# Transconnectome/multimodal_neuroimage

Measured on NVIDIA B200. Metric: window_attn_fwd_bwd, higher is better.
Workload: dtype bf16

## Files before the change

### multimodal_neuroimage_b200/csrc/tc_common.cuh

```cuda
#pragma once

#include <cuda.h>
#include <cuda_bf16.h>
#include <cuda_runtime.h>
#include <stdint.h>
#include <stdio.h>

namespace mmn { namespace tc {

__device__ __forceinline__ uint32_t smem_u32(const void* p) { return (uint32_t)__cvta_generic_to_shared(p); }

__device__ __forceinline__ void mbar_init(uint64_t* bar, uint32_t count) {
  asm volatile("mbarrier.init.shared::cta.b64 [%0], %1;" ::"r"(smem_u32(bar)), "r"(count));
}
__device__ __forceinline__ void fence_barrier_init() { asm volatile("fence.mbarrier_init.release.cluster;" ::: "memory"); }
__device__ __forceinline__ void mbar_arrive(uint64_t* bar) {
  asm volatile("mbarrier.arrive.shared::cta.b64 _, [%0];" ::"r"(smem_u32(bar)) : "memory");
}
__device__ __forceinline__ void mbar_arrive_warp(uint64_t* bar) {
  __syncwarp();
  if ((threadIdx.x & 31) == 0) mbar_arrive(bar);
}
__device__ __forceinline__ void mbar_arrive_expect_tx(uint64_t* bar, uint32_t bytes) {
  asm volatile("mbarrier.arrive.expect_tx.shared::cta.b64 _, [%0], %1;" ::"r"(smem_u32(bar)), "r"(bytes) : "memory");
}
__device__ __forceinline__ bool mbar_try_wait(uint64_t* bar, uint32_t parity) {
  uint32_t ok;
  asm volatile(
      "{\n\t.reg .pred p;\n\t"
      "mbarrier.try_wait.parity.shared::cta.b64 p, [%1], %2, %3;\n\t"
      "selp.u32 %0, 1, 0, p;\n\t}"
      : "=r"(ok)
      : "r"(smem_u32(bar)), "r"(parity), "r"(0x989680u)
      : "memory");
  return ok != 0;
}
__device__ __forceinline__ bool mbar_test(uint64_t* bar, uint32_t parity) {
  uint32_t ok;
  asm volatile(
      "{\n\t.reg .pred p;\n\t"
      "mbarrier.test_wait.parity.shared::cta.b64 p, [%1], %2;\n\t"
      "selp.u32 %0, 1, 0, p;\n\t}"
      : "=r"(ok)
      : "r"(smem_u32(bar)), "r"(parity)
      : "memory");
  return ok != 0;
}
__device__ __forceinline__ void mbar_wait(uint64_t* bar, uint32_t parity) {
  uint32_t spins = 0;
  while (!mbar_try_wait(bar, parity)) {
    if (++spins > (1u << 20)) {
#ifdef MMN_DEBUG_WAIT
      printf("mbar_wait timeout: block %d thread %d barrier smem 0x%x parity %u\n", (int)blockIdx.x, (int)threadIdx.x, smem_u32(bar), parity);
#endif
      __trap();
    }
  }
}

__device__ __forceinline__ bool elect_one() {
  uint32_t pred;
  asm volatile("{\n\t.reg .pred p;\n\telect.sync _|p, 0xffffffff;\n\tselp.u32 %0, 1, 0, p;\n\t}" : "=r"(pred));
  return pred != 0;
}

__device__ __forceinline__ void fence_proxy_async_smem() { asm volatile("fence.proxy.async.shared::cta;" ::: "memory"); }
__device__ __forceinline__ void tcgen05_fence_before() { asm volatile("tcgen05.fence::before_thread_sync;" ::: "memory"); }
__device__ __forceinline__ void tcgen05_fence_after() { asm volatile("tcgen05.fence::after_thread_sync;" ::: "memory"); }
__device__ __forceinline__ void named_bar_sync(uint32_t id, uint32_t threads) {
  asm volatile("bar.sync %0, %1;" ::"r"(id), "r"(threads) : "memory");
}

__device__ __forceinline__ void tma_prefetch_desc(const CUtensorMap* m) {
  asm volatile("prefetch.tensormap [%0];" ::"l"(reinterpret_cast<uint64_t>(m)) : "memory");
}
__device__ __forceinline__ void tma_load_5d(const CUtensorMap* m, uint64_t* bar, void* smem_dst, int c0, int c1, int c2,
                                            int c3, int c4) {
  asm volatile(
      "cp.async.bulk.tensor.5d.shared::cluster.global.mbarrier::complete_tx::bytes [%0], [%1, {%3, %4, %5, %6, %7}], [%2];"
      ::"r"(smem_u32(smem_dst)), "l"(reinterpret_cast<uint64_t>(m)), "r"(smem_u32(bar)), "r"(c0), "r"(c1), "r"(c2),
      "r"(c3), "r"(c4)
      : "memory");
}
__device__ __forceinline__ void tma_store_5d(const CUtensorMap* m, const void* smem_src, int c0, int c1, int c2, int c3,
                                             int c4) {
  asm volatile("cp.async.bulk.tensor.5d.global.shared::cta.bulk_group [%0, {%2, %3, %4, %5, %6}], [%1];" ::"l"(
                   reinterpret_cast<uint64_t>(m)),
               "r"(smem_u32(smem_src)), "r"(c0), "r"(c1), "r"(c2), "r"(c3), "r"(c4)
               : "memory");
}
__device__ __forceinline__ void tma_load_3d(const CUtensorMap* m, uint64_t* bar, void* smem_dst, int c0, int c1, int c2) {
  asm volatile(
      "cp.async.bulk.tensor.3d.shared::cluster.global.mbarrier::complete_tx::bytes [%0], [%1, {%3, %4, %5}], [%2];"
      ::"r"(smem_u32(smem_dst)), "l"(reinterpret_cast<uint64_t>(m)), "r"(smem_u32(bar)), "r"(c0), "r"(c1), "r"(c2)
      : "memory");
}
__device__ __forceinline__ void tma_load_4d(const CUtensorMap* m, uint64_t* bar, void* smem_dst, int c0, int c1, int c2, int c3) {
  asm volatile(
      "cp.async.bulk.tensor.4d.shared::cluster.global.mbarrier::complete_tx::bytes [%0], [%1, {%3, %4, %5, %6}], [%2];"
      ::"r"(smem_u32(smem_dst)), "l"(reinterpret_cast<uint64_t>(m)), "r"(smem_u32(bar)), "r"(c0), "r"(c1), "r"(c2), "r"(c3)
      : "memory");
}
__device__ __forceinline__ void tma_prefetch_3d(const CUtensorMap* m, int c0, int c1, int c2) {
  asm volatile("cp.async.bulk.prefetch.tensor.3d.L2.global.tile [%0, {%1, %2, %3}];" ::"l"(reinterpret_cast<uint64_t>(m)), "r"(c0),
               "r"(c1), "r"(c2)
               : "memory");
}
__device__ __forceinline__ void tma_store_3d(const CUtensorMap* m, const void* smem_src, int c0, int c1, int c2) {
  asm volatile("cp.async.bulk.tensor.3d.global.shared::cta.bulk_group [%0, {%2, %3, %4}], [%1];" ::"l"(
                   reinterpret_cast<uint64_t>(m)),
               "r"(smem_u32(smem_src)), "r"(c0), "r"(c1), "r"(c2)
               : "memory");
}
__device__ __forceinline__ void bulk_load_1d(void* smem_dst, const void* gsrc, uint32_t bytes, uint64_t* bar) {
  asm volatile("cp.async.bulk.shared::cluster.global.mbarrier::complete_tx::bytes [%0], [%1], %2, [%3];" ::"r"(smem_u32(smem_dst)),
               "l"(reinterpret_cast<uint64_t>(gsrc)), "r"(bytes), "r"(smem_u32(bar))
               : "memory");
}
__device__ __forceinline__ void tma_store_commit() { asm volatile("cp.async.bulk.commit_group;" ::: "memory"); }
template <int N>
__device__ __forceinline__ void tma_store_wait_read() { asm volatile("cp.async.bulk.wait_group.read %0;" ::"n"(N) : "memory"); }
template <int N>
__device__ __forceinline__ void tma_store_wait_all() { asm volatile("cp.async.bulk.wait_group %0;" ::"n"(N) : "memory"); }

template <int COLS>
__device__ __forceinline__ void tmem_alloc(uint32_t* dst_smem) {
  asm volatile("tcgen05.alloc.cta_group::1.sync.aligned.shared::cta.b32 [%0], %1;" ::"r"(smem_u32(dst_smem)), "n"(COLS)
               : "memory");
  asm volatile("tcgen05.relinquish_alloc_permit.cta_group::1.sync.aligned;" ::: "memory");
}
template <int COLS>
__device__ __forceinline__ void tmem_dealloc(uint32_t taddr) {
  asm volatile("tcgen05.dealloc.cta_group::1.sync.aligned.b32 %0, %1;" ::"r"(taddr), "n"(COLS) : "memory");
}
__device__ __forceinline__ void tmem_ld_wait() { asm volatile("tcgen05.wait::ld.sync.aligned;" ::: "memory"); }

__device__ __forceinline__ void tmem_ld_32x32b_x32(uint32_t taddr, uint32_t (&r)[32]) {
  asm volatile(
      "tcgen05.ld.sync.aligned.32x32b.x32.b32 "
      "{%0, %1, %2, %3, %4, %5, %6, %7, %8, %9, %10, %11, %12, %13, %14, %15, "
      "%16, %17, %18, %19, %20, %21, %22, %23, %24, %25, %26, %27, %28, %29, %30, %31}, [%32];"
      : "=r"(r[0]), "=r"(r[1]), "=r"(r[2]), "=r"(r[3]), "=r"(r[4]), "=r"(r[5]), "=r"(r[6]), "=r"(r[7]), "=r"(r[8]),
        "=r"(r[9]), "=r"(r[10]), "=r"(r[11]), "=r"(r[12]), "=r"(r[13]), "=r"(r[14]), "=r"(r[15]), "=r"(r[16]),
        "=r"(r[17]), "=r"(r[18]), "=r"(r[19]), "=r"(r[20]), "=r"(r[21]), "=r"(r[22]), "=r"(r[23]), "=r"(r[24]),
        "=r"(r[25]), "=r"(r[26]), "=r"(r[27]), "=r"(r[28]), "=r"(r[29]), "=r"(r[30]), "=r"(r[31])
      : "r"(taddr)
      : "memory");
}

__device__ __forceinline__ void tmem_ld_32x32b_x16(uint32_t taddr, uint32_t (&r)[16]) {
  asm volatile(
      "tcgen05.ld.sync.aligned.32x32b.x16.b32 "
      "{%0, %1, %2, %3, %4, %5, %6, %7, %8, %9, %10, %11, %12, %13, %14, %15}, [%16];"
      : "=r"(r[0]), "=r"(r[1]), "=r"(r[2]), "=r"(r[3]), "=r"(r[4]), "=r"(r[5]), "=r"(r[6]), "=r"(r[7]), "=r"(r[8]),
        "=r"(r[9]), "=r"(r[10]), "=r"(r[11]), "=r"(r[12]), "=r"(r[13]), "=r"(r[14]), "=r"(r[15])
      : "r"(taddr)
      : "memory");
}

__device__ __forceinline__ void tmem_ld_32x32b(uint32_t taddr, uint32_t (&r)[16]) { tmem_ld_32x32b_x16(taddr, r); }
__device__ __forceinline__ void tmem_ld_32x32b(uint32_t taddr, uint32_t (&r)[32]) { tmem_ld_32x32b_x32(taddr, r); }

__device__ __forceinline__ void tmem_st_32x32b_x32(uint32_t taddr, const uint32_t (&r)[32]) {
  asm volatile(
      "tcgen05.st.sync.aligned.32x32b.x32.b32 [%0], "
      "{%1, %2, %3, %4, %5, %6, %7, %8, %9, %10, %11, %12, %13, %14, %15, %16, "
      "%17, %18, %19, %20, %21, %22, %23, %24, %25, %26, %27, %28, %29, %30, %31, %32};"
      ::"r"(taddr), "r"(r[0]), "r"(r[1]), "r"(r[2]), "r"(r[3]), "r"(r[4]), "r"(r[5]), "r"(r[6]), "r"(r[7]), "r"(r[8]), "r"(r[9]),
      "r"(r[10]), "r"(r[11]), "r"(r[12]), "r"(r[13]), "r"(r[14]), "r"(r[15]), "r"(r[16]), "r"(r[17]), "r"(r[18]), "r"(r[19]),
      "r"(r[20]), "r"(r[21]), "r"(r[22]), "r"(r[23]), "r"(r[24]), "r"(r[25]), "r"(r[26]), "r"(r[27]), "r"(r[28]), "r"(r[29]),
      "r"(r[30]), "r"(r[31])
      : "memory");
}
__device__ __forceinline__ void tmem_st_32x32b_x16(uint32_t taddr, const uint32_t (&r)[16]) {
  asm volatile(
      "tcgen05.st.sync.aligned.32x32b.x16.b32 [%0], "
      "{%1, %2, %3, %4, %5, %6, %7, %8, %9, %10, %11, %12, %13, %14, %15, %16};"
      ::"r"(taddr), "r"(r[0]), "r"(r[1]), "r"(r[2]), "r"(r[3]), "r"(r[4]), "r"(r[5]), "r"(r[6]), "r"(r[7]), "r"(r[8]), "r"(r[9]),
      "r"(r[10]), "r"(r[11]), "r"(r[12]), "r"(r[13]), "r"(r[14]), "r"(r[15])
      : "memory");
}
__device__ __forceinline__ void tmem_st_wait() { asm volatile("tcgen05.wait::st.sync.aligned;" ::: "memory"); }

template <int R> __device__ __forceinline__ void setmaxnreg_inc() { asm volatile("setmaxnreg.inc.sync.aligned.u32 %0;" ::"n"(R)); }
template <int R> __device__ __forceinline__ void setmaxnreg_dec() { asm volatile("setmaxnreg.dec.sync.aligned.u32 %0;" ::"n"(R)); }

enum : uint64_t { kSwzNone = 0, kSwz128 = 2, kSwz64 = 4, kSwz32 = 6 };
__device__ __forceinline__ uint64_t umma_smem_desc(uint32_t saddr, uint32_t lbo_bytes, uint32_t sbo_bytes, uint64_t layout) {
  return (uint64_t)((saddr & 0x3FFFF) >> 4) | ((uint64_t)(lbo_bytes >> 4) << 16) | ((uint64_t)(sbo_bytes >> 4) << 32) |
         (1ull << 46) | (layout << 61);
}
__host__ __device__ constexpr uint32_t umma_idesc_bf16(int M, int N, int a_mn_major, int b_mn_major) {
  return (1u << 4) | (1u << 7) | (1u << 10) | ((uint32_t)a_mn_major << 15) | ((uint32_t)b_mn_major << 16) |
         ((uint32_t)(N >> 3) << 17) | ((uint32_t)(M >> 4) << 24);
}
__device__ __forceinline__ void umma_bf16_ss(uint32_t tmem_d, uint64_t adesc, uint64_t bdesc, uint32_t idesc, uint32_t accumulate) {
  asm volatile(
      "{\n\t.reg .pred p;\n\t"
      "setp.ne.b32 p, %4, 0;\n\t"
      "tcgen05.mma.cta_group::1.kind::f16 [%0], %1, %2, %3, p;\n\t}"
      ::"r"(tmem_d), "l"(adesc), "l"(bdesc), "r"(idesc), "r"(accumulate)
      : "memory");
}
__device__ __forceinline__ void umma_bf16_ts(uint32_t tmem_d, uint32_t tmem_a, uint64_t bdesc, uint32_t idesc, uint32_t accumulate) {
  asm volatile(
      "{\n\t.reg .pred p;\n\t"
      "setp.ne.b32 p, %4, 0;\n\t"
      "tcgen05.mma.cta_group::1.kind::f16 [%0], [%1], %2, %3, p;\n\t}"
      ::"r"(tmem_d), "r"(tmem_a), "l"(bdesc), "r"(idesc), "r"(accumulate)
      : "memory");
}
__device__ __forceinline__ void umma_commit(uint64_t* bar) {
  asm volatile("tcgen05.commit.cta_group::1.mbarrier::arrive::one.shared::cluster.b64 [%0];" ::"r"(smem_u32(bar)) : "memory");
}

__device__ __forceinline__ uint32_t pack_bf16x2(float lo, float hi) {
  __nv_bfloat162 v = __floats2bfloat162_rn(lo, hi);
  return *reinterpret_cast<uint32_t*>(&v);
}
__device__ __forceinline__ uint64_t pk2(float lo, float hi) {
  uint64_t r;
  asm("mov.b64 %0, {%1, %2};" : "=l"(r) : "f"(lo), "f"(hi));
  return r;
}
__device__ __forceinline__ uint64_t pk2u(uint32_t lo, uint32_t hi) {
  uint64_t r;
  asm("mov.b64 %0, {%1, %2};" : "=l"(r) : "r"(lo), "r"(hi));
  return r;
}
__device__ __forceinline__ void upk2(uint64_t v, float& lo, float& hi) { asm("mov.b64 {%0, %1}, %2;" : "=f"(lo), "=f"(hi) : "l"(v)); }
__device__ __forceinline__ uint64_t fma2(uint64_t a, uint64_t b, uint64_t c) {
  uint64_t r;
  asm("fma.rn.f32x2 %0, %1, %2, %3;" : "=l"(r) : "l"(a), "l"(b), "l"(c));
  return r;
}
__device__ __forceinline__ uint64_t mul2(uint64_t a, uint64_t b) {
  uint64_t r;
  asm("mul.rn.f32x2 %0, %1, %2;" : "=l"(r) : "l"(a), "l"(b));
  return r;
}
__device__ __forceinline__ uint64_t add2(uint64_t a, uint64_t b) {
  uint64_t r;
  asm("add.rn.f32x2 %0, %1, %2;" : "=l"(r) : "l"(a), "l"(b));
  return r;
}
__device__ __forceinline__ uint32_t pack_bf16x2(uint64_t v) {
  float lo, hi;
  upk2(v, lo, hi);
  return pack_bf16x2(lo, hi);
}
__device__ __forceinline__ float fast_exp2(float x) {
  float y;
  asm("ex2.approx.ftz.f32 %0, %1;" : "=f"(y) : "f"(x));
  return y;
}

}}
```

### multimodal_neuroimage_b200/csrc/winattn_tc_bwd.cuh

```cuda
#pragma once

#include "winattn_tc_fwd.cuh"

namespace mmn { namespace tc {

constexpr int kStagesB = 3;
constexpr int kStageBytesB = 2 * kQRegion + 2 * kTile;
constexpr int kOffK = kQRegion, kOffV = kQRegion + kTile, kOffDO = kQRegion + 2 * kTile;
#ifndef MMN_BWD_KEYS_PER_THREAD
#define MMN_BWD_KEYS_PER_THREAD 16
#endif
constexpr int kKeysPerThread = MMN_BWD_KEYS_PER_THREAD;
constexpr int kRowSplit = kN / kKeysPerThread;
constexpr int kSoftmaxThreadsB = 128 * kRowSplit, kEpiThreads = 128;
constexpr int kEpiWarp0 = kSoftmaxThreadsB / 32, kProducerWarpB = kEpiWarp0 + 4, kMmaWarpB = kEpiWarp0 + 5, kStoreWarpB = kEpiWarp0 + 6;
constexpr int kColsumWarpB = kEpiWarp0 + 7;
constexpr int kBwdThreads = kSoftmaxThreadsB + 256;
constexpr int kRegLaunch = kRowSplit == 4 ? 80 : 128;
constexpr int kRegSoftmax = kRowSplit == 4 ? 80 : 168, kRegEpi = kRowSplit == 4 ? 104 : 112, kRegAux = kRowSplit == 4 ? 56 : 64;
#ifndef MMN_BWD_CHUNK
#define MMN_BWD_CHUNK 1
#endif
constexpr int kChunkB = MMN_BWD_CHUNK;
constexpr int kPDBytes = 7 * 8192;
constexpr int kBwdTmemCols = 512;

struct BwdParams {
  CUtensorMap q[8], k[8], v[8], dout[8], dq[8], dk[8], dv[8];
  WinShape S;
  Sched sc;
  int nH, per_head;
  int mask_windows;
  float scale;
  const float* bias;
  const float* head_scale;
  const float* mask;
  const float* lse;
  long long slab;
  float* dbias;
  float* dhead_scale;
  float* dcolsum;
  int* work;
  float* part;
  TraceCfg trace;
};


constexpr int kDetColsum = kN * kN, kDetHscale = kN * kN + 3 * kD, kDetSlotFloats = kN * kN + 3 * kD + 4;

template <bool COS, int MASK, bool DET>
__global__ void __launch_bounds__(kBwdThreads, 1)
winattn_bwd_tc_kernel(const __grid_constant__ BwdParams P) {
  extern __shared__ uint8_t smem_raw[];
  uint8_t* smem = smem_raw + ((1024u - (smem_u32(smem_raw) & 1023u)) & 1023u);
  uint8_t* sStage = smem;
  uint8_t* sPD = sStage + kStagesB * kStageBytesB;
  uint8_t* sDS = sPD + 2 * 8192;
  uint8_t* sOut = sPD + kPDBytes;
  float* sTbl = reinterpret_cast<float*>(sOut + 3 * kTile);
  float* sRec = sTbl + kN * kTblLd;
  float* sDelta = sRec + kStagesB * 2 * 3 * kN;
  float* sRed = sDelta + 512;
  uint8_t* sPos = reinterpret_cast<uint8_t*>(sRed + 16);
  uint8_t* sRid = sPos + 512;
  int4* sItem = reinterpret_cast<int4*>(sRid + 512);
  int4* sGeo = sItem + 8;
  int* sEnd = reinterpret_cast<int*>(sGeo + 16);
  uint64_t* bars = reinterpret_cast<uint64_t*>(sEnd + 4);
  uint64_t* full = bars;
  uint64_t* empty = bars + kStagesB;
  uint64_t* sdp_full = bars + 2 * kStagesB;
  uint64_t* sdp_empty = sdp_full + 2;
  uint64_t* pds_full = sdp_full + 4;
  uint64_t* out_full = sdp_full + 5;
  uint64_t* out_empty = sdp_full + 7;
  uint64_t* so_ready = sdp_full + 9;
  uint64_t* so_free = sdp_full + 12;
  uint32_t* tmem_slot = reinterpret_cast<uint32_t*>(sdp_full + 15);

  const WinShape& S = P.S;
  const Sched& sc = P.sc;
  const int tid = threadIdx.x, warp = tid >> 5, lane = tid & 31;
  const int h = blockIdx.x % P.nH;
  float* const det_slot = DET ? P.part + (size_t)(h * P.per_head + blockIdx.x / P.nH) * kDetSlotFloats : nullptr;

  for (int i = tid; i < (kStagesB * kStageBytesB + kPDBytes) / 16; i += kBwdThreads)
    reinterpret_cast<uint4*>(smem)[i] = make_uint4(0, 0, 0, 0);
  for (int i = tid; i < 512; i += kBwdThreads) {
    sPos[i] = (uint8_t)piece_position(S, i >> 6, i & 63);
    sRid[i] = (uint8_t)class_region_id(S, i >> 6, i & 63);
  }
  for (int i = tid; i < kStagesB * 2 * 3 * kN; i += kBwdThreads) sRec[i] = 0.f;
  if (tid == 0) {
    sEnd[0] = 0x7fffffff;
    for (int s = 0; s < kStagesB; ++s) { mbar_init(&full[s], 1); mbar_init(&empty[s], kEpiThreads / 32); }
    for (int b = 0; b < 2; ++b) {
      mbar_init(&sdp_full[b], 1); mbar_init(&sdp_empty[b], kSoftmaxThreadsB / 32);
      mbar_init(&out_full[b], 1); mbar_init(&out_empty[b], kEpiThreads / 32);
    }
    mbar_init(pds_full, kSoftmaxThreadsB / 32);
    for (int t = 0; t < 3; ++t) { mbar_init(&so_ready[t], kEpiThreads / 32); mbar_init(&so_free[t], P.dcolsum ? 2 : 1); }
    fence_barrier_init();
  }
  if (warp == kProducerWarpB && lane == 0)
    for (int i = 0; i < 8; ++i) { tma_prefetch_desc(&P.q[i]); tma_prefetch_desc(&P.k[i]); tma_prefetch_desc(&P.v[i]); tma_prefetch_desc(&P.dout[i]); }
  if (warp == kStoreWarpB && lane == 0)
    for (int i = 0; i < 8; ++i) { tma_prefetch_desc(&P.dq[i]); tma_prefetch_desc(&P.dk[i]); tma_prefetch_desc(&P.dv[i]); }
  if (warp == kMmaWarpB) tmem_alloc<kBwdTmemCols>(tmem_slot);
  fence_proxy_async_smem();
  tcgen05_fence_before();
  __syncthreads();
  tcgen05_fence_after();
  const uint32_t tmem = *tmem_slot;
  trace_cta_time(P.trace, 0);

  if (warp >= kProducerWarpB) {
    setmaxnreg_dec<kRegAux>();
    if (warp == kProducerWarpB) {
      const CUtensorMap* const maps[4] = {P.q, P.dout, P.k, P.v};
      const int dst_base[4] = {0, kOffDO, kOffK, kOffV};
      const int slot_stride[4] = {2 * kWinBytes, 2 * kWinBytes, kWinBytes, kWinBytes};
      BoxPlan<4> plan;
      int n = 0;
#define MMN_BWD_LOAD_ITEM(cur)                                                                                           \
  do {                                                                                                                 \
    const int stage = n % kStagesB, phase = (n / kStagesB) & 1;                                                       \
    if ((cur).cls != plan.cls) plan.build(S, (cur).cls, lane, maps, dst_base, slot_stride);                           \
    const int nvalid = (cur).slot_valid(1) ? 2 : 1;                                                                   \
    int w0, w1;                                                                                                       \
    const WinStart ws0 = cursor_start(S, cur, 0, w0), ws1 = cursor_start(S, cur, 1, w1);                              \
    trace_ev(P.trace, 2, n, 0);                                                                                       \
    mbar_wait(&empty[stage], phase ^ 1);                                                                              \
    trace_ev(P.trace, 2, n, 1);                                                                                       \
    if (lane == 0) {                                                                                                  \
      sItem[n & 7] = make_int4((cur).cls, w0, w1, nvalid);                                                          \
      sGeo[(n & 7) * 2] = make_int4(ws0.b, ws0.s0, ws0.s1, ws0.s2);                                                   \
      sGeo[(n & 7) * 2 + 1] = make_int4(ws1.b, ws1.s0, ws1.s1, ws1.s2);                                               \
      mbar_arrive_expect_tx(&full[stage], nvalid * (4 * kWinBytes + 3 * kN * 4));                                     \
    }                                                                                                                 \
    __syncwarp();                                                                                                     \
    plan.issue<true>(S, ws0, ws1, nvalid, h * kD, sStage + stage * kStageBytesB, &full[stage], lane);                 \
    if (lane < nvalid)                                                                                                \
      bulk_load_1d(sRec + (stage * 2 + lane) * (3 * kN), P.lse + P.slab + ((long long)(lane ? w1 : w0) * P.nH + h) * (3 * kN),\
                   3 * kN * 4, &full[stage]);                                                                         \
    trace_ev(P.trace, 2, n, 2);                                                                                       \
  } while (0)
      if (DET) {
        const int k = blockIdx.x / P.nH, end = sched_range_begin(sc, k + 1, P.per_head);
        int it = sched_range_begin(sc, k, P.per_head);
        ItemCursor cur;
        cur.seek(sc, it);
        for (; it < end; ++it, ++n, cur.next_item(sc)) MMN_BWD_LOAD_ITEM(cur);
      } else {
        ClassQueue wq;
        wq.init(sc, sched_range_begin(sc, blockIdx.x / P.nH, P.per_head), P.work + h * 8, kChunkB, lane);
        for (int c0, m; wq.next(sc, P.work + h * 8, kChunkB, lane, c0, m);) {
          ItemCursor cur;
          cur.seek(sc, c0);
          for (int t = 0; t < m; ++t, ++n, cur.next_item(sc)) MMN_BWD_LOAD_ITEM(cur);
        }
      }
#undef MMN_BWD_LOAD_ITEM
      {
        const int stage = n % kStagesB, phase = (n / kStagesB) & 1;
        mbar_wait(&empty[stage], phase ^ 1);
        if (lane == 0) {
          sItem[n & 7] = make_int4(-1, 0, 0, 0);
          mbar_arrive(&full[stage]);
        }
        __syncwarp();
      }
    } else if (warp == kMmaWarpB) {
      constexpr uint32_t idescS = umma_idesc_bf16(128, 64, 0, 0);
      constexpr uint32_t idescKM = umma_idesc_bf16(128, 32, 0, 1);
      constexpr uint32_t idescMM = umma_idesc_bf16(128, 32, 1, 1);
      const uint64_t dKm = umma_smem_desc(0, 0, 512, kSwz64);
      const uint64_t dMn = umma_smem_desc(0, 8192, 512, kSwz64);
      const uint64_t dPk = umma_smem_desc(0, 0, 1024, kSwz128);
      const uint64_t dPm = umma_smem_desc(0, 8192, 1024, kSwz128);
      const uint32_t stage0 = smem_u32(sStage) >> 4, pd0 = smem_u32(sPD) >> 4, ds0 = smem_u32(sDS) >> 4;
      constexpr uint32_t W16 = kWinBytes >> 4;
      int total = 0x7fffffff;
      auto issue_sdp = [&](int n) {
        const int stage = n % kStagesB, phase = (n / kStagesB) & 1, b = n & 1;
        mbar_wait(&full[stage], phase);
        if (sItem[n & 7].x < 0) { total = n; return; }
        mbar_wait(&sdp_empty[b], ((n >> 1) & 1) ^ 1);
        tcgen05_fence_after();
        trace_ev(P.trace, 3, n - 2, 4);
        if (elect_one()) {
          const uint64_t sb = dKm + (stage0 + stage * (kStageBytesB >> 4));
          const uint32_t tS = tmem + b * 128, tDP = tS + 64;
#pragma unroll
          for (int ks = 0; ks < 4; ++ks)
            umma_bf16_ss(tS, sb + ((ks >> 1) * W16 + (ks & 1) * 2), sb + ((kOffK >> 4) + (ks >> 1) * W16 + (ks & 1) * 2), idescS, ks);
#pragma unroll
          for (int ks = 0; ks < 4; ++ks)
            umma_bf16_ss(tDP, sb + ((kOffDO >> 4) + (ks >> 1) * W16 + (ks & 1) * 2), sb + ((kOffV >> 4) + (ks >> 1) * W16 + (ks & 1) * 2), idescS, ks);
          umma_commit(&sdp_full[b]);
        }
        __syncwarp();
        trace_ev(P.trace, 3, n - 2, 5);
      };
      issue_sdp(0);
      if (total > 1) issue_sdp(1);
      for (int n = 0; n < total; ++n) {
        const int stage = n % kStagesB, b = n & 1;
        trace_ev(P.trace, 3, n, 0);
        mbar_wait(pds_full, n & 1);
        mbar_wait(&out_empty[b], ((n >> 1) & 1) ^ 1);
        trace_ev(P.trace, 3, n, 1);
        tcgen05_fence_after();
        if (elect_one()) {
          const uint64_t sbm = dMn + (stage0 + stage * (kStageBytesB >> 4));
          const uint64_t adk = dPk + ds0, adm = dPm + ds0;
          const uint64_t ap0 = umma_smem_desc(0, 3 * 8192 - b * 8192, 1024, kSwz128) + (pd0 + b * (8192 >> 4));
          const uint64_t ap1 = umma_smem_desc(0, 2 * 8192 + b * 8192, 1024, kSwz128) + (pd0 + ((3 * 8192) >> 4));
          const uint32_t tO = tmem + 256 + b * 96;
#pragma unroll
          for (int ks = 0; ks < 8; ++ks) {
            const uint32_t wofs = (ks >> 2) * 2 * W16 + (ks & 3) * 64;
            umma_bf16_ss(tO, (ks < 4 ? ap0 : ap1) + (ks & 3) * 128, sbm + ((kOffDO >> 4) + wofs), idescMM, ks);
            umma_bf16_ss(tO + 32, adk + ((ks >> 2) * 512 + (ks & 3) * 2), sbm + ((kOffK >> 4) + ks * 64), idescKM, ks);
            umma_bf16_ss(tO + 64, adm + ks * 128, sbm + wofs, idescMM, ks);
          }
          umma_commit(&out_full[b]);
        }
        __syncwarp();
        trace_ev(P.trace, 3, n, 2);
        if (total == 0x7fffffff) issue_sdp(n + 2);
        trace_ev(P.trace, 3, n, 3);
      }
      if (total >= 2) mbar_wait(&out_empty[total & 1], ((total - 2) >> 1) & 1);
      if (lane == 0) {
        sEnd[0] = total;
        mbar_arrive(&out_full[total & 1]);
      }
      __syncwarp();
    } else if (warp == kStoreWarpB) {
      const CUtensorMap* const maps[1] = {P.dq};
      const int dst_base[1] = {0};
      const int slot_stride[1] = {kWinBytes};
      BoxPlan<1> plan;
      int grp = 0;
      bool done = false;
      for (int n = 0; !done; ++n) {
        WinStart w0, w1;
        int nvalid = 0;
#pragma unroll
        for (int t = 0; t < 3; ++t, ++grp) {
          if (t == 0) trace_ev(P.trace, 4, n, 0);
          mbar_wait(&so_ready[t], n & 1);
          if (t == 0) {
            if (n >= *reinterpret_cast<volatile int*>(sEnd)) { done = true; break; }
            const int4 it = sItem[n & 7], a0 = sGeo[(n & 7) * 2], a1 = sGeo[(n & 7) * 2 + 1];
            nvalid = it.w;
            if (it.x != plan.cls) plan.build(S, it.x, lane, maps, dst_base, slot_stride);
            w0.b = a0.x; w0.s0 = a0.y; w0.s1 = a0.z; w0.s2 = a0.w;
            w1.b = a1.x; w1.s0 = a1.y; w1.s1 = a1.z; w1.s2 = a1.w;
            trace_ev(P.trace, 4, n, 1);
          }
          plan.issue<false>(S, w0, w1, nvalid, h * kD, sOut + t * kTile, nullptr, lane, 8 * t);
          tma_store_commit();
          tma_store_wait_read<2>();
          __syncwarp();
          if (lane == 0 && grp >= 2) mbar_arrive(&so_free[(t + 1) % 3]);
        }
        trace_ev(P.trace, 4, n, 2);
      }
      tma_store_wait_all<0>();
    } else if (warp == kColsumWarpB && P.dcolsum) {
      const int cg = lane & 3, r0 = lane >> 2;
      float acc[3][8];
#pragma unroll
      for (int t = 0; t < 3; ++t)
#pragma unroll
        for (int e = 0; e < 8; ++e) acc[t][e] = 0.f;
      bool done = false;
      for (int n = 0; !done; ++n) {
#pragma unroll
        for (int t = 0; t < 3; ++t) {
          mbar_wait(&so_ready[t], n & 1);
          if (t == 0 && n >= *reinterpret_cast<volatile int*>(sEnd)) { done = true; break; }
          const uint8_t* tile = sOut + t * kTile;
#pragma unroll 4
          for (int it = 0; it < 16; ++it) {
            const int row = r0 + 8 * it;
            const uint4 v = *reinterpret_cast<const uint4*>(tile + row * 64 + ((cg ^ ((row >> 1) & 3)) << 4));
            const uint32_t u[4] = {v.x, v.y, v.z, v.w};
#pragma unroll
            for (int e = 0; e < 4; ++e) {
              acc[t][2 * e] += __uint_as_float(u[e] << 16);
              acc[t][2 * e + 1] += __uint_as_float(u[e] & 0xffff0000u);
            }
          }
          __syncwarp();
          if (lane == 0) mbar_arrive(&so_free[t]);
        }
      }
      const int C = P.nH * kD;
#pragma unroll
      for (int t = 0; t < 3; ++t)
#pragma unroll
        for (int e = 0; e < 8; ++e) {
          float v = acc[t][e];
          v += __shfl_xor_sync(0xffffffffu, v, 4);
          v += __shfl_xor_sync(0xffffffffu, v, 8);
          v += __shfl_xor_sync(0xffffffffu, v, 16);
          if (lane < 4) {
            if (DET) det_slot[kDetColsum + t * kD + cg * 8 + e] = v;
            else atomicAdd(P.dcolsum + t * C + h * kD + cg * 8 + e, v);
          }
        }
    }
  } else if (warp >= kEpiWarp0) {
    const int r = tid - kEpiWarp0 * 32;
    const int slot = r >> 6, i = r & 63;
    const uint32_t lane_base = (uint32_t)((warp & 3) * 32) << 16;
    const int rsw = (r >> 1) & 3;
    if (kRegEpi > kRegLaunch) setmaxnreg_inc<kRegEpi>(); else if (kRegEpi < kRegLaunch) setmaxnreg_dec<kRegEpi>();
    float dscale_acc = 0.f;
    const float inv_hscale = COS ? 1.f / __ldg(P.head_scale + h) : 1.f;
    int n = 0;
    for (;; ++n) {
      const int stage = n % kStagesB, b = n & 1;
      const uint8_t* base = sStage + stage * kStageBytesB;
      const uint32_t tO = tmem + lane_base + 256 + b * 96;
      if (warp == kEpiWarp0) trace_ev(P.trace, 1, n, 0);
      mbar_wait(&out_full[b], (n >> 1) & 1);
      if (n >= *reinterpret_cast<volatile int*>(sEnd)) break;
      tcgen05_fence_after();
      const bool valid = slot < sItem[n & 7].w;
      if (warp == kEpiWarp0) trace_ev(P.trace, 1, n, 1);

      uint4 xrow[2][4];
      float rinv2[2] = {1.f, 1.f};
      if (COS) {
        const uint8_t* qrow = base + slot * 2 * kWinBytes + i * 64;
        const uint8_t* krow_ = base + kOffK + r * 64;
#pragma unroll
        for (int c = 0; c < 4; ++c) {
          xrow[0][c] = *reinterpret_cast<const uint4*>(qrow + ((c ^ rsw) << 4));
          xrow[1][c] = *reinterpret_cast<const uint4*>(krow_ + ((c ^ rsw) << 4));
        }
        rinv2[0] = sRec[(stage * 2 + slot) * (3 * kN) + i];
        rinv2[1] = sRec[(stage * 2 + slot) * (3 * kN) + kN + i];
      }
      mbar_arrive_warp(&empty[stage]);

#pragma unroll
      for (int t = 0; t < 3; ++t) {
        uint32_t g32[32];
        tmem_ld_32x32b_x32(tO + (t == 2 ? 0 : 32 + t * 32), g32);
        tmem_ld_wait();
        if (t == 2) {
          tcgen05_fence_before();
          mbar_arrive_warp(&out_empty[b]);
        }
        uint32_t o[16];
        if (COS && t < 2) {
          uint64_t x2[16];
          uint64_t dot2[4] = {0ull, 0ull, 0ull, 0ull};
#pragma unroll
          for (int c = 0; c < 4; ++c) {
            const uint4 xq = xrow[t][c];
            const uint32_t u[4] = {xq.x, xq.y, xq.z, xq.w};
#pragma unroll
            for (int e = 0; e < 4; ++e) {
              x2[c * 4 + e] = pk2u(u[e] << 16, u[e] & 0xffff0000u);
              dot2[e] = fma2(x2[c * 4 + e], pk2u(g32[c * 8 + 2 * e], g32[c * 8 + 2 * e + 1]), dot2[e]);
            }
          }
          const float rinv = rinv2[t];
          float xga, xgb;
          upk2(add2(add2(dot2[0], dot2[1]), add2(dot2[2], dot2[3])), xga, xgb);
          const float xg = xga + xgb;
          if (t == 0 && valid) dscale_acc += xg;
          const float proj = rinv >= 1e12f ? 0.f : -xg * rinv * rinv;
          const uint64_t proj2 = pk2(proj, proj);
#pragma unroll
          for (int c = 0; c < 16; ++c) {
            const uint64_t o2 = fma2(x2[c], proj2, pk2u(g32[2 * c], g32[2 * c + 1]));
            float o0, o1;
            upk2(o2, o0, o1);
            o[c] = pack_bf16x2(o0, o1);
          }
        } else {
#pragma unroll
          for (int c = 0; c < 16; ++c) o[c] = pack_bf16x2(__uint_as_float(g32[2 * c]), __uint_as_float(g32[2 * c + 1]));
        }
        mbar_wait(&so_free[t], (n & 1) ^ 1);
        uint8_t* orow = sOut + t * kTile + r * 64;
#pragma unroll
        for (int c = 0; c < 4; ++c)
          *reinterpret_cast<uint4*>(orow + ((c ^ rsw) << 4)) =
              valid ? make_uint4(o[c * 4 + 0], o[c * 4 + 1], o[c * 4 + 2], o[c * 4 + 3]) : make_uint4(0, 0, 0, 0);
        fence_proxy_async_smem();
        mbar_arrive_warp(&so_ready[t]);
        if (warp == kEpiWarp0) trace_ev(P.trace, 1, n, 2 + t);
      }
    }
    if (n > 0) mbar_wait(&so_free[0], (n - 1) & 1);
    mbar_arrive_warp(&so_ready[0]);
    if (COS && P.dhead_scale) {
#pragma unroll
      for (int o = 16; o > 0; o >>= 1) dscale_acc += __shfl_xor_sync(0xffffffffu, dscale_acc, o);
      if (lane == 0) {
        if (DET) det_slot[kDetHscale + (warp - kEpiWarp0)] = dscale_acc * inv_hscale;
        else atomicAdd(P.dhead_scale + h, dscale_acc * inv_hscale);
      }
    }
  } else {
    if (kRegSoftmax > kRegLaunch) setmaxnreg_inc<kRegSoftmax>();
    constexpr int KP = kKeysPerThread;
    const int r = tid & 127, qt = tid >> 7;
    const int slot = r >> 6, i = r & 63;
    const uint32_t lane_base = (uint32_t)((warp & 3) * 32) << 16;
    const float hscale = COS ? __ldg(P.head_scale + h) : P.scale;
    const float* bias_h = P.bias ? P.bias + (size_t)h * kN * kN : nullptr;
    float* const gdb_head = P.dbias ? P.dbias + (size_t)h * kN * kN : nullptr;
    uint8_t* prow0 = sPD + slot * (5 * 8192) + i * 128;
    uint8_t* drow = sDS + slot * 16384 + i * 128;
    float dbacc[KP];
#pragma unroll
    for (int j = 0; j < KP; ++j) dbacc[j] = 0.f;
    const int trole = warp == 0 ? 0 : -1;
    bool det_flushed = false;
#define TRB(item, ev) do { if (trole >= 0) trace_ev(P.trace, trole, item, ev); } while (0)

    auto flush_dbias = [&](int cls) {
      float4* mine = reinterpret_cast<float4*>(sTbl + i * kTblLd + qt * KP);
      if (slot == 0) {
#pragma unroll
        for (int j4 = 0; j4 < KP / 4; ++j4) mine[j4] = make_float4(dbacc[j4 * 4], dbacc[j4 * 4 + 1], dbacc[j4 * 4 + 2], dbacc[j4 * 4 + 3]);
      }
      named_bar_sync(3, kSoftmaxThreadsB);
      if (slot == 1) {
#pragma unroll
        for (int j4 = 0; j4 < KP / 4; ++j4) {
          float4 v = mine[j4];
          v.x += dbacc[j4 * 4]; v.y += dbacc[j4 * 4 + 1]; v.z += dbacc[j4 * 4 + 2]; v.w += dbacc[j4 * 4 + 3];
          mine[j4] = v;
        }
      }
#pragma unroll
      for (int j = 0; j < KP; ++j) dbacc[j] = 0.f;
      named_bar_sync(3, kSoftmaxThreadsB);
      const uint8_t* pos = sPos + cls * 64;
      for (int e = tid; e < kN * kN; e += kSoftmaxThreadsB) {
        const int ti = e >> 6, tj = e & 63;
        if (DET) {
          float* dst = det_slot + (int)pos[ti] * kN + pos[tj];
          *dst = (det_flushed ? *dst : 0.f) + sTbl[ti * kTblLd + tj];
        } else {
          atomicAdd(gdb_head + (int)pos[ti] * kN + pos[tj], sTbl[ti * kTblLd + tj]);
        }
      }
      det_flushed = true;
    };

    int cls_loaded = -1;
    for (int n = 0;; ++n) {
      const int b = n & 1, stage = n % kStagesB;
      TRB(n, 0);
      mbar_wait(&full[stage], (n / kStagesB) & 1);
      const int4 item = sItem[n & 7];
      if (item.x < 0) break;
      const int cls = item.x;
      const bool valid = slot < item.w;
      const float* rec = sRec + (stage * 2 + slot) * (3 * kN);
      const float lse2 = valid ? rec[2 * kN + i] : 0.f;
      if (cls != cls_loaded) {
        named_bar_sync(3, kSoftmaxThreadsB);
        if (gdb_head && cls_loaded >= 0) {
          flush_dbias(cls_loaded);
          named_bar_sync(3, kSoftmaxThreadsB);
        }
        build_class_table(sTbl, kTblLd, bias_h, sPos + cls * 64, sRid + cls * 64, MASK == MMN_MASK_SHIFT && cls != 0, tid, kSoftmaxThreadsB);
        cls_loaded = cls;
        named_bar_sync(3, kSoftmaxThreadsB);
      }
      TRB(n, 2);
      const float a_i = COS ? rec[i] * hscale : hscale;
      const float a_l2 = a_i * kLog2e;
      const float4* krow = reinterpret_cast<const float4*>(rec + kN + qt * KP);

      float p[KP];
      {
        const float4* trow = reinterpret_cast<const float4*>(sTbl + i * kTblLd + qt * KP);
        const float* mrow = nullptr;
        if (MASK == MMN_MASK_TENSOR) {
          const int gw = slot ? item.z : item.y, ipos = sPos[cls * 64 + i];
          mrow = P.mask + ((size_t)(gw % P.mask_windows) * kN + ipos) * kN + qt * KP;
        }
#pragma unroll
        for (int j4 = 0; j4 < KP / 4; ++j4) {
          float4 tt = trow[j4];
          if (MASK == MMN_MASK_TENSOR) {
            const float4 mm = __ldg(reinterpret_cast<const float4*>(mrow) + j4);
            tt.x = fmaf(mm.x, kLog2e, tt.x); tt.y = fmaf(mm.y, kLog2e, tt.y); tt.z = fmaf(mm.z, kLog2e, tt.z); tt.w = fmaf(mm.w, kLog2e, tt.w);
          }
          p[j4 * 4 + 0] = tt.x - lse2; p[j4 * 4 + 1] = tt.y - lse2; p[j4 * 4 + 2] = tt.z - lse2; p[j4 * 4 + 3] = tt.w - lse2;
        }
      }

      TRB(n, 3);
      mbar_wait(&sdp_full[b], (n >> 1) & 1);
      tcgen05_fence_after();
      TRB(n, 4);
      float delta = 0.f;
      {
        uint32_t raw[KP], dpr[KP];
        tmem_ld_32x32b(tmem + lane_base + b * 128 + qt * KP, raw);
        tmem_ld_32x32b(tmem + lane_base + b * 128 + 64 + qt * KP, dpr);
        tmem_ld_wait();
#pragma unroll
        for (int j4 = 0; j4 < KP / 4; ++j4) {
          const float4 kk = COS ? krow[j4] : make_float4(1.f, 1.f, 1.f, 1.f);
          const float rk[4] = {kk.x, kk.y, kk.z, kk.w};
#pragma unroll
          for (int e = 0; e < 4; ++e) {
            const int j = j4 * 4 + e;
            const float pj = fast_exp2(fmaf(__uint_as_float(raw[j]), COS ? rk[e] * a_l2 : a_l2, p[j]));
            const float dpj = __uint_as_float(dpr[j]);
            delta = fmaf(pj, dpj, delta);
            p[j] = pj;
          }
        }
      }
      sDelta[qt * 128 + r] = delta;
      TRB(n, 5);
      if (n > 1) mbar_wait(&out_full[b], ((n - 2) >> 1) & 1);
      uint8_t* prow = prow0 + b * 8192;
      TRB(n, 6);
#pragma unroll
      for (int c = 0; c < KP / 8; ++c) {
        uint4 v4 = make_uint4(pack_bf16x2(p[c * 8 + 0], p[c * 8 + 1]), pack_bf16x2(p[c * 8 + 2], p[c * 8 + 3]),
                              pack_bf16x2(p[c * 8 + 4], p[c * 8 + 5]), pack_bf16x2(p[c * 8 + 6], p[c * 8 + 7]));
        if (!valid) v4 = make_uint4(0, 0, 0, 0);
        *reinterpret_cast<uint4*>(prow + (((qt * (KP / 8) + c) ^ (i & 7)) << 4)) = v4;
      }
      named_bar_sync(2, kSoftmaxThreadsB);
      TRB(n, 7);
      delta = sDelta[r] + sDelta[128 + r];
      if (kRowSplit == 4) delta += sDelta[256 + r] + sDelta[384 + r];

      {
        uint32_t dpr[KP];
        tmem_ld_32x32b(tmem + lane_base + b * 128 + 64 + qt * KP, dpr);
        tmem_ld_wait();
        tcgen05_fence_before();
        mbar_arrive_warp(&sdp_empty[b]);
#pragma unroll
        for (int j = 0; j < KP; ++j) p[j] *= __uint_as_float(dpr[j]) - delta;
      }
      if (valid && gdb_head) {
#pragma unroll
        for (int j = 0; j < KP; ++j) dbacc[j] += p[j];
      }
      if (n > 0) mbar_wait(&out_full[b ^ 1], ((n - 1) >> 1) & 1);
#pragma unroll
      for (int c = 0; c < KP / 8; ++c) {
        float cj[8];
        if (COS) {
          const float4 k0 = krow[c * 2], k1 = krow[c * 2 + 1];
          cj[0] = k0.x * a_i; cj[1] = k0.y * a_i; cj[2] = k0.z * a_i; cj[3] = k0.w * a_i;
          cj[4] = k1.x * a_i; cj[5] = k1.y * a_i; cj[6] = k1.z * a_i; cj[7] = k1.w * a_i;
        } else {
#pragma unroll
          for (int e = 0; e < 8; ++e) cj[e] = a_i;
        }
        uint4 v4 = make_uint4(pack_bf16x2(p[c * 8 + 0] * cj[0], p[c * 8 + 1] * cj[1]), pack_bf16x2(p[c * 8 + 2] * cj[2], p[c * 8 + 3] * cj[3]),
                              pack_bf16x2(p[c * 8 + 4] * cj[4], p[c * 8 + 5] * cj[5]), pack_bf16x2(p[c * 8 + 6] * cj[6], p[c * 8 + 7] * cj[7]));
        if (!valid) v4 = make_uint4(0, 0, 0, 0);
        *reinterpret_cast<uint4*>(drow + (((qt * (KP / 8) + c) ^ (i & 7)) << 4)) = v4;
      }
      fence_proxy_async_smem();
      mbar_arrive_warp(pds_full);
      TRB(n, 8);
    }
#undef TRB

    if (gdb_head && cls_loaded >= 0) {
      named_bar_sync(3, kSoftmaxThreadsB);
      flush_dbias(cls_loaded);
    } else if (DET && gdb_head) {
      for (int e = tid; e < kN * kN; e += kSoftmaxThreadsB) det_slot[e] = 0.f;
    }
  }

  tcgen05_fence_before();
  __syncthreads();
  trace_cta_time(P.trace, 1);
  if (warp == kMmaWarpB) tmem_dealloc<kBwdTmemCols>(tmem);
}

constexpr size_t kBwdSmemBytes = 1024 + kStagesB * kStageBytesB + kPDBytes + 3 * kTile + kN * kTblLd * 4 +
                                 (kStagesB * 2 * 3 * kN + 512 + 16) * 4 + 1024 + 24 * 16 + 16 + 24 * 8;

constexpr int kDetRedSlices = 32;
__global__ void __launch_bounds__(kDetRedSlices * 32)
winattn_bwd_det_reduce(const float* __restrict__ part, int per_head, int nH, float* __restrict__ dbias, float* __restrict__ dcolsum,
                       float* __restrict__ dhead_scale) {
  __shared__ float4 red[kDetRedSlices][32];
  const int lane = threadIdx.x & 31, sl = threadIdx.x >> 5, h = blockIdx.y;
  const int e = (blockIdx.x * 32 + lane) * 4;
  const float* base = part + (size_t)h * per_head * kDetSlotFloats;
  float4 acc = make_float4(0.f, 0.f, 0.f, 0.f);
  if (e < kDetSlotFloats) {
#pragma unroll 4
    for (int k = sl; k < per_head; k += kDetRedSlices) {
      const float4 v = __ldg(reinterpret_cast<const float4*>(base + (size_t)k * kDetSlotFloats + e));
      acc.x += v.x; acc.y += v.y; acc.z += v.z; acc.w += v.w;
    }
  }
  red[sl][lane] = acc;
  __syncthreads();
  if (sl < 4) {
    acc = red[8 * sl][lane];
#pragma unroll
    for (int k = 1; k < 8; ++k) { const float4 v = red[8 * sl + k][lane]; acc.x += v.x; acc.y += v.y; acc.z += v.z; acc.w += v.w; }
    red[8 * sl][lane] = acc;
  }
  __syncthreads();
  if (sl != 0 || e >= kDetSlotFloats) return;
#pragma unroll
  for (int k = 1; k < 4; ++k) { const float4 v = red[8 * k][lane]; acc.x += v.x; acc.y += v.y; acc.z += v.z; acc.w += v.w; }
  if (e < kDetColsum) {
    if (dbias) {
      float4* o = reinterpret_cast<float4*>(dbias + (size_t)h * kN * kN + e);
      float4 r = *o;
      r.x += acc.x; r.y += acc.y; r.z += acc.z; r.w += acc.w;
      *o = r;
    }
  } else if (e < kDetHscale) {
    if (dcolsum) {
      const int t = (e - kDetColsum) / kD, c = (e - kDetColsum) % kD;
      float* o = dcolsum + (size_t)t * nH * kD + h * kD + c;
      o[0] += acc.x; o[1] += acc.y; o[2] += acc.z; o[3] += acc.w;
    }
  } else if (dhead_scale) {
    dhead_scale[h] += (acc.x + acc.y) + (acc.z + acc.w);
  }
}

inline int bwd_ctas_per_head(const WinShape& S, const mmn_winattn_desc* d) {
  int per_head = num_sms_cached() / d->num_heads;
  if (per_head < 1) per_head = 1;
  const int n_items = make_sched(S, d->batch, true).n_items;
  return per_head > n_items ? n_items : per_head;
}

inline size_t bwd_det_workspace_bytes_impl(const mmn_winattn_desc* d) {
  return (size_t)bwd_ctas_per_head(shape_from(d), d) * d->num_heads * kDetSlotFloats * sizeof(float);
}

inline const char* bwd_why_not_impl(const mmn_winattn_desc* d) {
  const char* w = fwd_why_not_impl(d);
  if (w) return w;
  if (d->do_row_stride % 8 || d->dq_row_stride % 8 || d->dk_row_stride % 8 || d->dv_row_stride % 8) return "gradient row stride not 16-byte aligned";
  return nullptr;
}

inline int winattn_bwd_launch(const mmn_winattn_desc* d, const void* q, const void* k, const void* v, const float* bias,
                              const float* head_scale, const float* mask, const float* lse, const void* dout, void* dq, void* dk,
                              void* dv, float* dbias, float* dhead_scale, float* dcolsum, void* workspace, cudaStream_t st, char* err, size_t errlen,
                              int* launches) {
  BwdParams P;
  P.S = shape_from(d);
  P.sc = make_sched(P.S, d->batch, true);
  const int C = d->num_heads * d->head_dim;
  const int B = d->batch;
  if (!make_window_maps(P.q, q, d->q_row_stride, B, C, P.S) || !make_window_maps(P.k, k, d->k_row_stride, B, C, P.S) ||
      !make_window_maps(P.v, v, d->v_row_stride, B, C, P.S) || !make_window_maps(P.dout, dout, d->do_row_stride, B, C, P.S) ||
      !make_window_maps(P.dq, dq, d->dq_row_stride, B, C, P.S) || !make_window_maps(P.dk, dk, d->dk_row_stride, B, C, P.S) ||
      !make_window_maps(P.dv, dv, d->dv_row_stride, B, C, P.S)) {
    snprintf(err, errlen, "cuTensorMapEncodeTiled failed (pointer alignment or strides)");
    return MMN_ERR_CUDA;
  }
  P.nH = d->num_heads;
  P.mask_windows = d->mask_windows > 0 ? d->mask_windows : 1;
  P.scale = d->scale;
  P.bias = bias; P.head_scale = head_scale; P.mask = mask; P.lse = lse;
  P.slab = (long long)P.S.n_windows * d->num_heads * kN;
  P.dbias = bias ? dbias : nullptr;
  P.dhead_scale = d->score_kind == MMN_SCORE_COSINE ? dhead_scale : nullptr;
  P.dcolsum = dcolsum;
  const bool det = d->deterministic != 0;
  P.work = nullptr;
  P.part = nullptr;
  if (det) {
    if (!workspace || reinterpret_cast<uintptr_t>(workspace) % 16) { snprintf(err, errlen, "workspace missing or misaligned"); return MMN_ERR_CUDA; }
    P.part = static_cast<float*>(workspace);
  } else {
    P.work = arm_work_counters(workspace, st, err, errlen);
    if (!P.work) return MMN_ERR_CUDA;
  }
  const char* trace_path = getenv("MMN_TC_TRACE_BWD");
  P.trace = trace_setup(trace_path, st);

  using Kern = void (*)(const BwdParams);
  static const Kern kernels[2][2][3] = {
      {{winattn_bwd_tc_kernel<false, MMN_MASK_NONE, false>, winattn_bwd_tc_kernel<false, MMN_MASK_SHIFT, false>, winattn_bwd_tc_kernel<false, MMN_MASK_TENSOR, false>},
       {winattn_bwd_tc_kernel<true, MMN_MASK_NONE, false>, winattn_bwd_tc_kernel<true, MMN_MASK_SHIFT, false>, winattn_bwd_tc_kernel<true, MMN_MASK_TENSOR, false>}},
      {{winattn_bwd_tc_kernel<false, MMN_MASK_NONE, true>, winattn_bwd_tc_kernel<false, MMN_MASK_SHIFT, true>, winattn_bwd_tc_kernel<false, MMN_MASK_TENSOR, true>},
       {winattn_bwd_tc_kernel<true, MMN_MASK_NONE, true>, winattn_bwd_tc_kernel<true, MMN_MASK_SHIFT, true>, winattn_bwd_tc_kernel<true, MMN_MASK_TENSOR, true>}}};
  static std::once_flag once;
  std::call_once(once, [] {
    for (int t = 0; t < 2; ++t)
      for (int c = 0; c < 2; ++c)
        for (int m = 0; m < 3; ++m) cudaFuncSetAttribute(kernels[t][c][m], cudaFuncAttributeMaxDynamicSharedMemorySize, (int)kBwdSmemBytes);
  });
  const Kern kern = kernels[det ? 1 : 0][d->score_kind == MMN_SCORE_COSINE ? 1 : 0][d->mask_kind];
  P.per_head = bwd_ctas_per_head(P.S, d);
  kern<<<P.per_head * P.nH, kBwdThreads, kBwdSmemBytes, st>>>(P);
  cudaError_t e = cudaGetLastError();
  if (e != cudaSuccess) {
    snprintf(err, errlen, "winattn_bwd_tc_kernel: %s", cudaGetErrorString(e));
    return MMN_ERR_CUDA;
  }
  ++*launches;
  if (det && (P.dbias || P.dhead_scale || P.dcolsum)) {
    winattn_bwd_det_reduce<<<dim3((kDetSlotFloats / 4 + 31) / 32, P.nH), kDetRedSlices * 32, 0, st>>>(P.part, P.per_head, P.nH, P.dbias,
                                                                                                    P.dcolsum, P.dhead_scale);
    e = cudaGetLastError();
    if (e != cudaSuccess) {
      snprintf(err, errlen, "winattn_bwd_det_reduce: %s", cudaGetErrorString(e));
      return MMN_ERR_CUDA;
    }
    ++*launches;
  }
  if (P.trace.buf) dump_trace(P.trace.buf, trace_path, st);
  return MMN_OK;
}

}}
```

Before: 264.7.

## Move bwd bias/mask class table into TMEM and drop softmax-group barriers

Each softmax thread now stores its own row slice of the per-class bias/mask table into spare TMEM columns and reads it back with tcgen05.ld, replacing the shared-memory table that was built cooperatively and guarded by named barriers. This frees the table's shared memory, and dbias reduction now reuses the P/dS buffers. The stage-empty barrier also gets an extra arrival from the MMA warp's commit, so the epilogue can read its COS rows and release the stage before waiting on out_full. The risks are TMEM column pressure and subtle ordering issues when reusing the P/dS buffers for the dbias flush.

Result: slower. 258.8, median of 6 (-2.2%).

```diff
diff --git a/multimodal_neuroimage_b200/csrc/tc_common.cuh b/multimodal_neuroimage_b200/csrc/tc_common.cuh
--- a/multimodal_neuroimage_b200/csrc/tc_common.cuh
+++ b/multimodal_neuroimage_b200/csrc/tc_common.cuh
@@ -180,6 +180,8 @@
       "r"(r[10]), "r"(r[11]), "r"(r[12]), "r"(r[13]), "r"(r[14]), "r"(r[15])
       : "memory");
 }
+__device__ __forceinline__ void tmem_st_32x32b(uint32_t taddr, const uint32_t (&r)[16]) { tmem_st_32x32b_x16(taddr, r); }
+__device__ __forceinline__ void tmem_st_32x32b(uint32_t taddr, const uint32_t (&r)[32]) { tmem_st_32x32b_x32(taddr, r); }
 __device__ __forceinline__ void tmem_st_wait() { asm volatile("tcgen05.wait::st.sync.aligned;" ::: "memory"); }
 
 template <int R> __device__ __forceinline__ void setmaxnreg_inc() { asm volatile("setmaxnreg.inc.sync.aligned.u32 %0;" ::"n"(R)); }
diff --git a/multimodal_neuroimage_b200/csrc/winattn_tc_bwd.cuh b/multimodal_neuroimage_b200/csrc/winattn_tc_bwd.cuh
--- a/multimodal_neuroimage_b200/csrc/winattn_tc_bwd.cuh
+++ b/multimodal_neuroimage_b200/csrc/winattn_tc_bwd.cuh
@@ -24,6 +24,7 @@
 constexpr int kChunkB = MMN_BWD_CHUNK;
 constexpr int kPDBytes = 7 * 8192;
 constexpr int kBwdTmemCols = 512;
+constexpr int kTblCol = 448;
 
 struct BwdParams {
   CUtensorMap q[8], k[8], v[8], dout[8], dq[8], dk[8], dv[8];
@@ -57,8 +58,7 @@
   uint8_t* sPD = sStage + kStagesB * kStageBytesB;
   uint8_t* sDS = sPD + 2 * 8192;
   uint8_t* sOut = sPD + kPDBytes;
-  float* sTbl = reinterpret_cast<float*>(sOut + 3 * kTile);
-  float* sRec = sTbl + kN * kTblLd;
+  float* sRec = reinterpret_cast<float*>(sOut + 3 * kTile);
   float* sDelta = sRec + kStagesB * 2 * 3 * kN;
   float* sRed = sDelta + 512;
   uint8_t* sPos = reinterpret_cast<uint8_t*>(sRed + 16);
@@ -93,7 +93,7 @@
   for (int i = tid; i < kStagesB * 2 * 3 * kN; i += kBwdThreads) sRec[i] = 0.f;
   if (tid == 0) {
     sEnd[0] = 0x7fffffff;
-    for (int s = 0; s < kStagesB; ++s) { mbar_init(&full[s], 1); mbar_init(&empty[s], kEpiThreads / 32); }
+    for (int s = 0; s < kStagesB; ++s) { mbar_init(&full[s], 1); mbar_init(&empty[s], kEpiThreads / 32 + 1); }
     for (int b = 0; b < 2; ++b) {
       mbar_init(&sdp_full[b], 1); mbar_init(&sdp_empty[b], kSoftmaxThreadsB / 32);
       mbar_init(&out_full[b], 1); mbar_init(&out_empty[b], kEpiThreads / 32);
@@ -225,6 +225,7 @@
             umma_bf16_ss(tO + 64, adm + ks * 128, sbm + wofs, idescMM, ks);
           }
           umma_commit(&out_full[b]);
+          umma_commit(&empty[stage]);
         }
         __syncwarp();
         trace_ev(P.trace, 3, n, 2);
@@ -327,26 +328,27 @@
       const uint8_t* base = sStage + stage * kStageBytesB;
       const uint32_t tO = tmem + lane_base + 256 + b * 96;
       if (warp == kEpiWarp0) trace_ev(P.trace, 1, n, 0);
+      mbar_wait(&full[stage], (n / kStagesB) & 1);
+      const int4 item = sItem[n & 7];
+      uint4 xrow[2][4];
+      float rinv2[2] = {1.f, 1.f};
+      if (COS && item.x >= 0) {
+        const uint8_t* qrow = base + slot * 2 * kWinBytes + i * 64;
+        const uint8_t* krow_ = base + kOffK + r * 64;
+#pragma unroll
+        for (int c = 0; c < 4; ++c) {
+          xrow[0][c] = *reinterpret_cast<const uint4*>(qrow + ((c ^ rsw) << 4));
+          xrow[1][c] = *reinterpret_cast<const uint4*>(krow_ + ((c ^ rsw) << 4));
+        }
+        rinv2[0] = sRec[(stage * 2 + slot) * (3 * kN) + i];
+        rinv2[1] = sRec[(stage * 2 + slot) * (3 * kN) + kN + i];
+      }
+      if (item.x >= 0) mbar_arrive_warp(&empty[stage]);
       mbar_wait(&out_full[b], (n >> 1) & 1);
       if (n >= *reinterpret_cast<volatile int*>(sEnd)) break;
       tcgen05_fence_after();
-      const bool valid = slot < sItem[n & 7].w;
+      const bool valid = slot < item.w;
       if (warp == kEpiWarp0) trace_ev(P.trace, 1, n, 1);
-
-      uint4 xrow[2][4];
-      float rinv2[2] = {1.f, 1.f};
-      if (COS) {
-        const uint8_t* qrow = base + slot * 2 * kWinBytes + i * 64;
-        const uint8_t* krow_ = base + kOffK + r * 64;
-#pragma unroll
-        for (int c = 0; c < 4; ++c) {
-          xrow[0][c] = *reinterpret_cast<const uint4*>(qrow + ((c ^ rsw) << 4));
-          xrow[1][c] = *reinterpret_cast<const uint4*>(krow_ + ((c ^ rsw) << 4));
-        }
-        rinv2[0] = sRec[(stage * 2 + slot) * (3 * kN) + i];
-        rinv2[1] = sRec[(stage * 2 + slot) * (3 * kN) + kN + i];
-      }
-      mbar_arrive_warp(&empty[stage]);
 
 #pragma unroll
       for (int t = 0; t < 3; ++t) {
@@ -428,8 +430,27 @@
     bool det_flushed = false;
 #define TRB(item, ev) do { if (trole >= 0) trace_ev(P.trace, trole, item, ev); } while (0)
 
-    auto flush_dbias = [&](int cls) {
-      float4* mine = reinterpret_cast<float4*>(sTbl + i * kTblLd + qt * KP);
+    const uint32_t ttbl = tmem + lane_base + kTblCol + qt * KP;
+    auto load_table = [&](int cls) {
+      const uint8_t* pos = sPos + cls * 64;
+      const uint8_t* rid = sRid + cls * 64;
+      const bool shift_mask = MASK == MMN_MASK_SHIFT && cls != 0;
+      const int pi = pos[i], ri = rid[pi];
+      uint32_t tv[KP];
+#pragma unroll
+      for (int j = 0; j < KP; ++j) {
+        const int pj = pos[qt * KP + j];
+        float v = bias_h ? __ldg(bias_h + pi * kN + pj) : 0.f;
+        if (shift_mask && rid[pj] != ri) v -= 100.f;
+        tv[j] = __float_as_uint(v * 1.4426950408889634f);
+      }
+      tmem_st_32x32b(ttbl, tv);
+      tmem_st_wait();
+    };
+
+    auto flush_dbias = [&](int cls, int pb) {
+      auto red_row = [&](int row) { return reinterpret_cast<float*>(sPD + (row >> 5) * (5 * 8192) + pb * 8192) + (row & 31) * kN; };
+      float4* mine = reinterpret_cast<float4*>(red_row(i) + qt * KP);
       if (slot == 0) {
 #pragma unroll
         for (int j4 = 0; j4 < KP / 4; ++j4) mine[j4] = make_float4(dbacc[j4 * 4], dbacc[j4 * 4 + 1], dbacc[j4 * 4 + 2], dbacc[j4 * 4 + 3]);
@@ -451,16 +472,18 @@
         const int ti = e >> 6, tj = e & 63;
         if (DET) {
           float* dst = det_slot + (int)pos[ti] * kN + pos[tj];
-          *dst = (det_flushed ? *dst : 0.f) + sTbl[ti * kTblLd + tj];
+          *dst = (det_flushed ? *dst : 0.f) + red_row(ti)[tj];
         } else {
-          atomicAdd(gdb_head + (int)pos[ti] * kN + pos[tj], sTbl[ti * kTblLd + tj]);
+          atomicAdd(gdb_head + (int)pos[ti] * kN + pos[tj], red_row(ti)[tj]);
         }
       }
       det_flushed = true;
+      named_bar_sync(3, kSoftmaxThreadsB);
     };
 
     int cls_loaded = -1;
-    for (int n = 0;; ++n) {
+    int n = 0;
+    for (;; ++n) {
       const int b = n & 1, stage = n % kStagesB;
       TRB(n, 0);
       mbar_wait(&full[stage], (n / kStagesB) & 1);
@@ -471,14 +494,12 @@
       const float* rec = sRec + (stage * 2 + slot) * (3 * kN);
       const float lse2 = valid ? rec[2 * kN + i] : 0.f;
       if (cls != cls_loaded) {
-        named_bar_sync(3, kSoftmaxThreadsB);
         if (gdb_head && cls_loaded >= 0) {
-          flush_dbias(cls_loaded);
-          named_bar_sync(3, kSoftmaxThreadsB);
-        }
-        build_class_table(sTbl, kTblLd, bias_h, sPos + cls * 64, sRid + cls * 64, MASK == MMN_MASK_SHIFT && cls != 0, tid, kSoftmaxThreadsB);
+          if (n > 1) mbar_wait(&out_full[b], ((n - 2) >> 1) & 1);
+          flush_dbias(cls_loaded, b);
+        }
+        load_table(cls);
         cls_loaded = cls;
-        named_bar_sync(3, kSoftmaxThreadsB);
       }
       TRB(n, 2);
       const float a_i = COS ? rec[i] * hscale : hscale;
@@ -487,20 +508,23 @@
 
       float p[KP];
       {
-        const float4* trow = reinterpret_cast<const float4*>(sTbl + i * kTblLd + qt * KP);
+        uint32_t tt[KP];
+        tmem_ld_32x32b(ttbl, tt);
         const float* mrow = nullptr;
         if (MASK == MMN_MASK_TENSOR) {
           const int gw = slot ? item.z : item.y, ipos = sPos[cls * 64 + i];
           mrow = P.mask + ((size_t)(gw % P.mask_windows) * kN + ipos) * kN + qt * KP;
         }
+        tmem_ld_wait();
 #pragma unroll
         for (int j4 = 0; j4 < KP / 4; ++j4) {
-          float4 tt = trow[j4];
+          float4 t4 = make_float4(__uint_as_float(tt[j4 * 4]), __uint_as_float(tt[j4 * 4 + 1]), __uint_as_float(tt[j4 * 4 + 2]),
+                                  __uint_as_float(tt[j4 * 4 + 3]));
           if (MASK == MMN_MASK_TENSOR) {
             const float4 mm = __ldg(reinterpret_cast<const float4*>(mrow) + j4);
-            tt.x = fmaf(mm.x, kLog2e, tt.x); tt.y = fmaf(mm.y, kLog2e, tt.y); tt.z = fmaf(mm.z, kLog2e, tt.z); tt.w = fmaf(mm.w, kLog2e, tt.w);
+            t4.x = fmaf(mm.x, kLog2e, t4.x); t4.y = fmaf(mm.y, kLog2e, t4.y); t4.z = fmaf(mm.z, kLog2e, t4.z); t4.w = fmaf(mm.w, kLog2e, t4.w);
           }
-          p[j4 * 4 + 0] = tt.x - lse2; p[j4 * 4 + 1] = tt.y - lse2; p[j4 * 4 + 2] = tt.z - lse2; p[j4 * 4 + 3] = tt.w - lse2;
+          p[j4 * 4 + 0] = t4.x - lse2; p[j4 * 4 + 1] = t4.y - lse2; p[j4 * 4 + 2] = t4.z - lse2; p[j4 * 4 + 3] = t4.w - lse2;
         }
       }
 
@@ -559,6 +583,7 @@
         for (int j = 0; j < KP; ++j) dbacc[j] += p[j];
       }
       if (n > 0) mbar_wait(&out_full[b ^ 1], ((n - 1) >> 1) & 1);
+      TRB(n, 9);
 #pragma unroll
       for (int c = 0; c < KP / 8; ++c) {
         float cj[8];
@@ -582,8 +607,8 @@
 #undef TRB
 
     if (gdb_head && cls_loaded >= 0) {
-      named_bar_sync(3, kSoftmaxThreadsB);
-      flush_dbias(cls_loaded);
+      mbar_wait(&out_full[(n - 1) & 1], ((n - 1) >> 1) & 1);
+      flush_dbias(cls_loaded, (n - 1) & 1);
     } else if (DET && gdb_head) {
       for (int e = tid; e < kN * kN; e += kSoftmaxThreadsB) det_slot[e] = 0.f;
     }
@@ -595,7 +620,7 @@
   if (warp == kMmaWarpB) tmem_dealloc<kBwdTmemCols>(tmem);
 }
 
-constexpr size_t kBwdSmemBytes = 1024 + kStagesB * kStageBytesB + kPDBytes + 3 * kTile + kN * kTblLd * 4 +
+constexpr size_t kBwdSmemBytes = 1024 + kStagesB * kStageBytesB + kPDBytes + 3 * kTile +
                                  (kStagesB * 2 * 3 * kN + 512 + 16) * 4 + 1024 + 24 * 16 + 16 + 24 * 8;
 
 constexpr int kDetRedSlices = 32;
```
